# marc345/Dense2Sparse-ViT

Hardware: AMD Instinct MI355X
Metric: training images/s, DeiT-S 224 keep_ratio=0.5 (dense-to-sparse ViT train step, teacher fwd + student fwd/bwd + AdamW) (higher is better)
Workload: dtype f32; 1 GPU; DeiT-Small 224x224 patch16, 1-stage prune keep_ratio=0.5 @ block 3 (196->98 tokens), large LN predictor, kl_div mask loss, per-GPU batch 128; global_batch=128, parallelism=dp1

## Files before the change

dense2sparse-vit_amd/csrc/attention_f32.hip:

```cpp
#include "d2s_common.h"

namespace {

#ifdef D2S_ATTN_STAMPS
__device__ unsigned long long g_attn_stamps[16 * 8192];
#define ASTAMP(i) if (threadIdx.x == 0) { const int L_ = blockIdx.y * gridDim.x + blockIdx.x; if (L_ < 8192) g_attn_stamps[16 * L_ + (i)] = __builtin_amdgcn_s_memtime(); }
#define ASTAMPR(i) if (threadIdx.x == 0) { const int L_ = blockIdx.y * gridDim.x + blockIdx.x; if (L_ < 8192) g_attn_stamps[16 * L_ + (i)] = __builtin_amdgcn_s_memrealtime(); }
#else
#define ASTAMP(i)
#define ASTAMPR(i)
#endif

constexpr int DH = 64;
constexpr int PITCH = 68;

__device__ __forceinline__ void load_rows_regs(const float* __restrict__ base, long ld, int row, int nrows, int half,
                                               float scale, f32x4 (&r)[8]) {
    if (row < nrows) {
        const float* p = base + (long)row * ld + 4 * half;
#pragma unroll
        for (int t = 0; t < 8; ++t) {
            r[t] = *reinterpret_cast<const f32x4*>(p + 8 * t);
#pragma unroll
            for (int j = 0; j < 4; ++j) r[t][j] *= scale;
        }
    } else {
#pragma unroll
        for (int t = 0; t < 8; ++t) r[t] = f32x4{0.f, 0.f, 0.f, 0.f};
    }
}

__device__ __forceinline__ void tile_load(const float* __restrict__ base, long ld, int row0, int nrows, int tid, f32x4 (&r)[2]) {
#pragma unroll
    for (int i = 0; i < 2; ++i) {
        const int f = tid + i * 256, row = row0 + (f >> 4), d4 = (f & 15) * 4;
        r[i] = row < nrows ? *reinterpret_cast<const f32x4*>(base + (long)row * ld + d4) : f32x4{0.f, 0.f, 0.f, 0.f};
    }
}
__device__ __forceinline__ void tile_store(float* __restrict__ S, int tid, const f32x4 (&r)[2]) {
#pragma unroll
    for (int i = 0; i < 2; ++i) {
        const int f = tid + i * 256;
        *reinterpret_cast<f32x4*>(&S[(f >> 4) * PITCH + (f & 15) * 4]) = r[i];
    }
}

__device__ __forceinline__ void mma_lds_reg(const float* __restrict__ S, int l31, int half, const f32x4 (&y)[8], f32x16& acc) {
#pragma unroll
    for (int t = 0; t < 8; ++t) {
        const f32x4 a = *reinterpret_cast<const f32x4*>(&S[l31 * PITCH + 8 * t + 4 * half]);
#pragma unroll
        for (int j = 0; j < 4; ++j) acc = mfma32(a[j], y[t][j], acc);
    }
}
__device__ __forceinline__ void mma_reg_lds(const f32x16& p, const float* __restrict__ S, int l31, int half, f32x16 (&o)[2],
                                            int groups = 4) {
#pragma unroll
    for (int g = 0; g < 4; ++g) {
        if (g < groups) {
#pragma unroll
            for (int r = 4 * g; r < 4 * g + 4; ++r) {
                const float* row = &S[mfma32_row(r, half) * PITCH];
                o[0] = mfma32(p[r], row[l31], o[0]);
                o[1] = mfma32(p[r], row[32 + l31], o[1]);
            }
        }
    }
}

__device__ __forceinline__ void mma_lds_reg_t(const f32x16& p, const float* __restrict__ S, int l31, int half, f32x16 (&o)[2],
                                              int groups = 4) {
#pragma unroll
    for (int g = 0; g < 4; ++g) {
        if (g < groups) {
#pragma unroll
            for (int r = 4 * g; r < 4 * g + 4; ++r) {
                const float* row = &S[mfma32_row(r, half) * PITCH];
                o[0] = mfma32(row[l31], p[r], o[0]);
                o[1] = mfma32(row[32 + l31], p[r], o[1]);
            }
        }
    }
}

struct AttnFwdArgs {
    const float* qkv; float* out; float* lse; float* cls_row;
    const float* policy; float* cinv; const int* cu;
    int n, H; float scale, eps; int total;
};

template <bool POLICY, bool VARLEN>
__global__ __launch_bounds__(256, 3) void attn_fwd_kernel(AttnFwdArgs a) {
    __shared__ __attribute__((aligned(16))) float Ks[32 * PITCH];
    __shared__ __attribute__((aligned(16))) float Vs[32 * PITCH];
    __shared__ float pol_s[32];
    __shared__ __attribute__((aligned(16))) float vred[POLICY ? 16 * 64 : 4];
    __shared__ float vsum_s[64];
    extern __shared__ __attribute__((aligned(16))) float cls_s[];
    const int tid = threadIdx.x, lane = tid & 63, wave = tid >> 6, half = lane >> 5, l31 = lane & 31;
    const int H = a.H;
    ASTAMP(0); ASTAMPR(8);
    int bx, by;
    xcd_remap_2d(bx, by);
    const int b = by / H, h = by % H;
    const long ld = 3L * H * DH;
    const int row_base = VARLEN ? a.cu[b] : 0;
    const int n = VARLEN ? a.cu[b + 1] - row_base : a.n;
    if (VARLEN && bx * 128 >= n) return;
    const long tok0 = VARLEN ? (long)row_base : (long)b * n;
    const float* qb = a.qkv + tok0 * ld + h * DH;
    const float* kb = qb + (long)H * DH;
    const float* vb = kb + (long)H * DH;
    const float* polb = POLICY ? a.policy + (long)b * n : nullptr;
    const float scale = a.scale;
    const int q0 = bx * 128 + wave * 32;
    const bool active = q0 < n;
    const bool want_cls = a.cls_row != nullptr && bx == 0 && wave == 0;
    const int qi = q0 + l31;

    f32x4 qreg[8];
    load_rows_regs(qb, ld, qi, n, half, scale, qreg);

    f32x16 o[2];
#pragma unroll
    for (int r = 0; r < 16; ++r) { o[0][r] = 0.f; o[1][r] = 0.f; }
    float m_run = -INFINITY, l_run = 0.f;
    f32x4 vacc = {0.f, 0.f, 0.f, 0.f};

    const int ntiles = (n + 31) / 32;
    f32x4 kr[2], vr[2];
    float pr = 0.f;
    tile_load(kb, ld, 0, n, tid, kr);
    tile_load(vb, ld, 0, n, tid, vr);
    if (POLICY && tid < 32) pr = tid < n ? polb[tid] : 0.f;
    for (int t = 0; t < ntiles; ++t) {
        __syncthreads();
        tile_store(Ks, tid, kr);
        tile_store(Vs, tid, vr);
        if (POLICY) {
            if (tid < 32) pol_s[tid] = pr;
            vacc += vr[0];
            vacc += vr[1];
        }
        __syncthreads();
        if (t == 0) { ASTAMP(1); }
        if (t == 1) { ASTAMP(2); }
        if (t == 2) { ASTAMP(3); }
        if (t + 1 < ntiles) {
            tile_load(kb, ld, (t + 1) * 32, n, tid, kr);
            tile_load(vb, ld, (t + 1) * 32, n, tid, vr);
            if (POLICY && tid < 32) { const int kj = (t + 1) * 32 + tid; pr = kj < n ? polb[kj] : 0.f; }
        }
        if (!active) continue;
        f32x16 s;
#pragma unroll
        for (int r = 0; r < 16; ++r) s[r] = 0.f;
        mma_lds_reg(Ks, l31, half, qreg, s);
        const int kv0 = t * 32;
        float mt = -INFINITY;
#pragma unroll
        for (int r = 0; r < 16; ++r) {
            if (kv0 + mfma32_row(r, half) >= n) s[r] = -INFINITY;
            mt = fmaxf(mt, s[r]);
        }
        if (want_cls && l31 == 0) {
#pragma unroll
            for (int r = 0; r < 16; ++r) {
                const int key = kv0 + mfma32_row(r, half);
                if (key < n) cls_s[key] = s[r];
            }
        }
        mt = fmaxf(mt, __shfl_xor(mt, 32, 64));
        const float m_new = fmaxf(m_run, mt);
        const float alpha = __expf(m_run - m_new);
        float rs = 0.f;
#pragma unroll
        for (int r = 0; r < 16; ++r) {
            s[r] = __expf(s[r] - m_new);
            if (POLICY) {
                const int kr_ = mfma32_row(r, half);
                s[r] *= (kv0 + kr_ == qi) ? 1.f : pol_s[kr_];
            }
            rs += s[r];
        }
        rs += __shfl_xor(rs, 32, 64);
        l_run = l_run * alpha + rs;
        m_run = m_new;
#pragma unroll
        for (int r = 0; r < 16; ++r) {
            o[0][r] *= alpha;
            o[1][r] *= alpha;
        }
        mma_lds_reg_t(s, Vs, l31, half, o, min(4, (n - kv0 + 7) >> 3));
    }
    ASTAMP(4);
    const float c = POLICY ? a.eps / (float)n : 0.f;
    if (POLICY) {
        *reinterpret_cast<f32x4*>(&vred[(tid >> 4) * 64 + (tid & 15) * 4]) = vacc;
        __syncthreads();
        if (tid < 64) {
            float t = 0.f;
#pragma unroll
            for (int g = 0; g < 16; ++g) t += vred[g * 64 + tid];
            vsum_s[tid] = t * c;
        }
        __syncthreads();
    }
    if (!active) return;
    const float inv_l = 1.0f / (POLICY ? l_run + a.eps : l_run);
    if (qi < n) {
        float* p = a.out + (tok0 + qi) * H * DH + h * DH;
#pragma unroll
        for (int dt = 0; dt < 2; ++dt)
#pragma unroll
            for (int g = 0; g < 4; ++g) {
                f32x4 v;
#pragma unroll
                for (int j = 0; j < 4; ++j) {
                    float num = o[dt][4 * g + j];
                    if (POLICY) num += vsum_s[32 * dt + 8 * g + 4 * half + j];
                    v[j] = num * inv_l;
                }
                *reinterpret_cast<f32x4*>(p + 32 * dt + 8 * g + 4 * half) = v;
            }
    }
    const long stat0 = VARLEN ? (long)h * a.total + row_base : ((long)b * H + h) * n;
    if (half == 0 && qi < n) {
        if (a.lse) a.lse[stat0 + qi] = m_run + logf(POLICY ? l_run + a.eps : l_run);
        if (POLICY && a.cinv) a.cinv[stat0 + qi] = c * inv_l;
    }
    if (want_cls) {
        const float m0 = __shfl(m_run, 0, 64), il0 = __shfl(inv_l, 0, 64);
        float* cr = a.cls_row + stat0;
        for (int j = lane; j < n; j += 64) {
            float e = expf(cls_s[j] - m0);
            if (POLICY) e = e * (j == 0 ? 1.f : polb[j]) + c;
            cr[j] = e * il0;
        }
    }
    ASTAMP(5); ASTAMPR(9);
}

__global__ __launch_bounds__(256) void attn_delta_kernel(const float* __restrict__ out, const float* __restrict__ dout,
                                                         float* __restrict__ delta, long rows, int n, int H) {
    const int lane = threadIdx.x & 63;
    const long row = (long)blockIdx.x * 4 + (threadIdx.x >> 6);
    if (row >= rows) return;
    const long b = row / n, i = row - b * n;
    for (int h = 0; h < H; ++h) {
        const long e = row * H * DH + h * DH + lane;
        const float s = wave_sum(out[e] * dout[e]);
        if (lane == 0) delta[(b * H + h) * n + i] = s;
    }
}

template <bool POLICY>
__global__ __launch_bounds__(256, 3) void attn_bwd_dq_kernel(const float* __restrict__ qkv, const float* __restrict__ dout,
                                                          const float* __restrict__ lse, const float* __restrict__ delta,
                                                          float* __restrict__ dqkv, int n, int H, float scale,
                                                          const float* __restrict__ policy) {
    __shared__ __attribute__((aligned(16))) float Ks[32 * PITCH];
    __shared__ __attribute__((aligned(16))) float Vs[32 * PITCH];
    __shared__ float pol_s[32];
    const int tid = threadIdx.x, lane = tid & 63, wave = tid >> 6, half = lane >> 5, l31 = lane & 31;
    int bx, by;
    xcd_remap_2d(bx, by);
    const int b = by / H, h = by % H;
    const long ld = 3L * H * DH, ldo = (long)H * DH;
    const float* qb = qkv + (long)b * n * ld + h * DH;
    const float* kb = qb + (long)H * DH;
    const float* vb = kb + (long)H * DH;
    const float* dob = dout + (long)b * n * ldo + h * DH;
    const int q0 = bx * 128 + wave * 32;
    const bool active = q0 < n;

    f32x4 qreg[8], doreg[8];
    load_rows_regs(qb, ld, q0 + l31, n, half, scale, qreg);
    load_rows_regs(dob, ldo, q0 + l31, n, half, 1.0f, doreg);
    const bool qok = q0 + l31 < n;
    const float lse_i = qok ? lse[((long)b * H + h) * n + q0 + l31] : INFINITY;
    const float dl_i = qok ? delta[((long)b * H + h) * n + q0 + l31] : 0.f;

    f32x16 dq[2];
#pragma unroll
    for (int r = 0; r < 16; ++r) { dq[0][r] = 0.f; dq[1][r] = 0.f; }

    const int ntiles = (n + 31) / 32;
    f32x4 kr[2], vr[2];
    float pr = 0.f;
    const float* polb = POLICY ? policy + (long)b * n : nullptr;
    tile_load(kb, ld, 0, n, tid, kr);
    tile_load(vb, ld, 0, n, tid, vr);
    if (POLICY && tid < 32) pr = tid < n ? polb[tid] : 0.f;
    for (int t = 0; t < ntiles; ++t) {
        __syncthreads();
        tile_store(Ks, tid, kr);
        tile_store(Vs, tid, vr);
        if (POLICY && tid < 32) pol_s[tid] = pr;
        __syncthreads();
        if (t + 1 < ntiles) {
            tile_load(kb, ld, (t + 1) * 32, n, tid, kr);
            tile_load(vb, ld, (t + 1) * 32, n, tid, vr);
            if (POLICY && tid < 32) { const int kj = (t + 1) * 32 + tid; pr = kj < n ? polb[kj] : 0.f; }
        }
        if (!active) continue;
        f32x16 s, dp;
#pragma unroll
        for (int r = 0; r < 16; ++r) { s[r] = 0.f; dp[r] = 0.f; }
        mma_lds_reg(Ks, l31, half, qreg, s);
        mma_lds_reg(Vs, l31, half, doreg, dp);
        const int kv0 = t * 32;
#pragma unroll
        for (int r = 0; r < 16; ++r) {
            const int kr_ = mfma32_row(r, half);
            float p = (kv0 + kr_ < n) ? __expf(s[r] - lse_i) : 0.f;
            if (POLICY) p *= (kv0 + kr_ == q0 + l31) ? 1.f : pol_s[kr_];
            s[r] = p * (dp[r] - dl_i);
        }
        mma_reg_lds(s, Ks, l31, half, dq, min(4, (n - kv0 + 7) >> 3));
    }
    if (!active) return;
    float* dqb = dqkv + (long)b * n * ld + h * DH;
#pragma unroll
    for (int r = 0; r < 16; ++r) {
        const int qi = q0 + mfma32_row(r, half);
        if (qi < n) {
            float* p = dqb + (long)qi * ld;
            p[l31] = dq[0][r] * scale;
            p[32 + l31] = dq[1][r] * scale;
        }
    }
}

template <bool POLICY>
__global__ __launch_bounds__(256, 2) void attn_bwd_dkv_kernel(const float* __restrict__ qkv, const float* __restrict__ dout,
                                                           const float* __restrict__ lse, const float* __restrict__ delta,
                                                           float* __restrict__ dqkv, int n, int H, float scale,
                                                           const float* __restrict__ policy, const float* __restrict__ cinv) {
    __shared__ __attribute__((aligned(16))) float Qs[32 * PITCH];
    __shared__ __attribute__((aligned(16))) float Ds[32 * PITCH];
    __shared__ float lse_s[32], dl_s[32], ci_s[32];
    const int tid = threadIdx.x, lane = tid & 63, wave = tid >> 6, half = lane >> 5, l31 = lane & 31;
    int bx, by;
    xcd_remap_2d(bx, by);
    const int b = by / H, h = by % H;
    const long ld = 3L * H * DH, ldo = (long)H * DH;
    const float* qb = qkv + (long)b * n * ld + h * DH;
    const float* kb = qb + (long)H * DH;
    const float* vb = kb + (long)H * DH;
    const float* dob = dout + (long)b * n * ldo + h * DH;
    const float* lse_b = lse + ((long)b * H + h) * n;
    const float* dl_b = delta + ((long)b * H + h) * n;
    const int k0 = bx * 128 + wave * 32;
    const bool active = k0 < n;

    f32x4 kreg[8], vreg[8];
    load_rows_regs(kb, ld, k0 + l31, n, half, scale, kreg);
    load_rows_regs(vb, ld, k0 + l31, n, half, 1.0f, vreg);

    f32x16 dk[2], dv[2];
#pragma unroll
    for (int r = 0; r < 16; ++r) { dk[0][r] = 0.f; dk[1][r] = 0.f; dv[0][r] = 0.f; dv[1][r] = 0.f; }

    const int ntiles = (n + 31) / 32;
    f32x4 qr[2], dr[2];
    float lr = 0.f, dlr = 0.f, cir = 0.f;
    const float* ci_b = POLICY ? cinv + ((long)b * H + h) * n : nullptr;
    const float pol_key = (POLICY && k0 + l31 < n) ? policy[(long)b * n + k0 + l31] : 0.f;
    tile_load(qb, ld, 0, n, tid, qr);
    tile_load(dob, ldo, 0, n, tid, dr);
    if (tid < 32) { lr = tid < n ? lse_b[tid] : INFINITY; dlr = tid < n ? dl_b[tid] : 0.f; if (POLICY) cir = tid < n ? ci_b[tid] : 0.f; }
    for (int t = 0; t < ntiles; ++t) {
        __syncthreads();
        tile_store(Qs, tid, qr);
        tile_store(Ds, tid, dr);
        if (tid < 32) { lse_s[tid] = lr; dl_s[tid] = dlr; if (POLICY) ci_s[tid] = cir; }
        __syncthreads();
        if (t + 1 < ntiles) {
            tile_load(qb, ld, (t + 1) * 32, n, tid, qr);
            tile_load(dob, ldo, (t + 1) * 32, n, tid, dr);
            if (tid < 32) {
                const int qi = (t + 1) * 32 + tid;
                lr = qi < n ? lse_b[qi] : INFINITY;
                dlr = qi < n ? dl_b[qi] : 0.f;
                if (POLICY) cir = qi < n ? ci_b[qi] : 0.f;
            }
        }
        if (!active) continue;
        f32x16 s, dp;
#pragma unroll
        for (int r = 0; r < 16; ++r) { s[r] = 0.f; dp[r] = 0.f; }
        mma_lds_reg(Qs, l31, half, kreg, s);
        mma_lds_reg(Ds, l31, half, vreg, dp);
#pragma unroll
        for (int r = 0; r < 16; ++r) {
            const int qi = mfma32_row(r, half);
            float p = __expf(s[r] - lse_s[qi]);
            if (POLICY) p *= (t * 32 + qi == k0 + l31) ? 1.f : pol_key;
            s[r] = POLICY ? p + ci_s[qi] : p;
            dp[r] = p * (dp[r] - dl_s[qi]);
        }
        const int qgroups = min(4, (n - t * 32 + 7) >> 3);
        mma_reg_lds(s, Ds, l31, half, dv, qgroups);
        mma_reg_lds(dp, Qs, l31, half, dk, qgroups);
    }
    if (!active) return;
    float* dkb = dqkv + (long)b * n * ld + (long)H * DH + h * DH;
    float* dvb = dkb + (long)H * DH;
#pragma unroll
    for (int r = 0; r < 16; ++r) {
        const int ki = k0 + mfma32_row(r, half);
        if (ki < n) {
            float* pk = dkb + (long)ki * ld;
            float* pv = dvb + (long)ki * ld;
            pk[l31] = dk[0][r] * scale;
            pk[32 + l31] = dk[1][r] * scale;
            pv[l31] = dv[0][r];
            pv[32 + l31] = dv[1][r];
        }
    }
}

}

#ifdef D2S_ATTN_STAMPS
extern "C" int d2s_debug_read_attn_stamps(unsigned long long* host_out, int n_wg) {
    return hipMemcpyFromSymbol(host_out, HIP_SYMBOL(g_attn_stamps), (size_t)n_wg * 16 * sizeof(unsigned long long)) == hipSuccess ? 0 : -1;
}
#endif

extern "C" {

int d2s_attn_fwd_f32(const float* qkv, float* out, float* lse, float* cls_row, int B, int n, int H, float scale,
                     hipStream_t stream) {
    if (!qkv || !out || !lse || B <= 0 || n <= 0 || H <= 0 || n > 8192) return D2S_ERR_ARG;
    dim3 grid((n + 127) / 128, B * H), block(256);
    AttnFwdArgs a{qkv, out, lse, cls_row, nullptr, nullptr, nullptr, n, H, scale, 0.f, 0};
    hipLaunchKernelGGL((attn_fwd_kernel<false, false>), grid, block, cls_row ? (size_t)n * sizeof(float) : 0, stream, a);
    return d2s_check_launch();
}

int d2s_attn_policy_fwd_f32(const float* qkv, const float* policy, float* out, float* lse, float* cinv, float* cls_row, int B, int n,
                            int H, float scale, float eps, hipStream_t stream) {
    if (!qkv || !policy || !out || !lse || !cinv || B <= 0 || n <= 0 || H <= 0 || n > 8192) return D2S_ERR_ARG;
    dim3 grid((n + 127) / 128, B * H), block(256);
    AttnFwdArgs a{qkv, out, lse, cls_row, policy, cinv, nullptr, n, H, scale, eps, 0};
    hipLaunchKernelGGL((attn_fwd_kernel<true, false>), grid, block, cls_row ? (size_t)n * sizeof(float) : 0, stream, a);
    return d2s_check_launch();
}

int d2s_attn_varlen_fwd_f32(const float* qkv, const int* cu_seqlens, float* out, float* cls_row, int B, int total, int max_n, int H,
                            float scale, hipStream_t stream) {
    if (!qkv || !cu_seqlens || !out || B <= 0 || total <= 0 || max_n <= 0 || max_n > 8192 || H <= 0) return D2S_ERR_ARG;
    dim3 grid((max_n + 127) / 128, B * H), block(256);
    AttnFwdArgs a{qkv, out, nullptr, cls_row, nullptr, nullptr, cu_seqlens, 0, H, scale, 0.f, total};
    hipLaunchKernelGGL((attn_fwd_kernel<false, true>), grid, block, cls_row ? (size_t)max_n * sizeof(float) : 0, stream, a);
    return d2s_check_launch();
}

int d2s_attn_delta(const float* out, const float* dout, float* delta, int B, int n, int H, hipStream_t stream) {
    if (!out || !dout || !delta || B <= 0 || n <= 0 || H <= 0) return D2S_ERR_ARG;
    const long rows = (long)B * n;
    hipLaunchKernelGGL(attn_delta_kernel, dim3((unsigned)((rows + 3) / 4)), dim3(256), 0, stream, out, dout, delta, rows, n, H);
    return d2s_check_launch();
}

int d2s_attn_bwd_f32(const float* qkv, const float* out, const float* dout, const float* lse, float* dqkv, float* delta_ws, int B,
                     int n, int H, float scale, hipStream_t stream) {
    if (!qkv || !out || !dout || !lse || !dqkv || !delta_ws || B <= 0 || n <= 0 || H <= 0) return D2S_ERR_ARG;
    const long rows = (long)B * n;
    hipLaunchKernelGGL(attn_delta_kernel, dim3((unsigned)((rows + 3) / 4)), dim3(256), 0, stream, out, dout, delta_ws, rows, n, H);
    dim3 grid((n + 127) / 128, B * H), block(256);
    hipLaunchKernelGGL(attn_bwd_dq_kernel<false>, grid, block, 0, stream, qkv, dout, lse, delta_ws, dqkv, n, H, scale,
                       static_cast<const float*>(nullptr));
    hipLaunchKernelGGL(attn_bwd_dkv_kernel<false>, grid, block, 0, stream, qkv, dout, lse, delta_ws, dqkv, n, H, scale,
                       static_cast<const float*>(nullptr), static_cast<const float*>(nullptr));
    return d2s_check_launch();
}

int d2s_attn_bwd_dq_f32(const float* qkv, const float* dout, const float* lse, const float* delta_ws, float* dqkv, int B, int n, int H,
                        float scale, hipStream_t stream) {
    if (!qkv || !dout || !lse || !dqkv || !delta_ws || B <= 0 || n <= 0 || H <= 0) return D2S_ERR_ARG;
    dim3 grid((n + 127) / 128, B * H), block(256);
    hipLaunchKernelGGL(attn_bwd_dq_kernel<false>, grid, block, 0, stream, qkv, dout, lse, delta_ws, dqkv, n, H, scale,
                       static_cast<const float*>(nullptr));
    return d2s_check_launch();
}
int d2s_attn_bwd_dkv_f32(const float* qkv, const float* dout, const float* lse, const float* delta_ws, float* dqkv, int B, int n, int H,
                         float scale, hipStream_t stream) {
    if (!qkv || !dout || !lse || !dqkv || !delta_ws || B <= 0 || n <= 0 || H <= 0) return D2S_ERR_ARG;
    dim3 grid((n + 127) / 128, B * H), block(256);
    hipLaunchKernelGGL(attn_bwd_dkv_kernel<false>, grid, block, 0, stream, qkv, dout, lse, delta_ws, dqkv, n, H, scale,
                       static_cast<const float*>(nullptr), static_cast<const float*>(nullptr));
    return d2s_check_launch();
}

int d2s_attn_policy_bwd_f32(const float* qkv, const float* policy, const float* out, const float* dout, const float* lse,
                            const float* cinv, float* dqkv, float* delta_ws, int B, int n, int H, float scale, hipStream_t stream) {
    if (!qkv || !policy || !out || !dout || !lse || !cinv || !dqkv || !delta_ws || B <= 0 || n <= 0 || H <= 0) return D2S_ERR_ARG;
    const long rows = (long)B * n;
    hipLaunchKernelGGL(attn_delta_kernel, dim3((unsigned)((rows + 3) / 4)), dim3(256), 0, stream, out, dout, delta_ws, rows, n, H);
    dim3 grid((n + 127) / 128, B * H), block(256);
    hipLaunchKernelGGL(attn_bwd_dq_kernel<true>, grid, block, 0, stream, qkv, dout, lse, delta_ws, dqkv, n, H, scale, policy);
    hipLaunchKernelGGL(attn_bwd_dkv_kernel<true>, grid, block, 0, stream, qkv, dout, lse, delta_ws, dqkv, n, H, scale, policy, cinv);
    return d2s_check_launch();
}

}
```

Before: 3594 images/s.

## Add single-block short-sequence attention fwd/bwd kernels for n<=256

Adds specialized attention kernels used when sequence length is at most 256 (the ViT case: 197 and 99 tokens). The forward launches one workgroup per (batch, head) with one wave per 32-query tile, sharing K/V tiles through LDS with register prefetch. The backward fuses the delta computation, dK/dV, and dQ into a single kernel that keeps all of K in LDS and assigns dQ chains to idle waves, replacing three launches and redundant K/Q reloads. It is enabled by default via an env toggle; the trade-off is fewer, larger workgroups (less grid parallelism) and high LDS use per block.

```diff
diff --git a/dense2sparse-vit_amd/csrc/attention_f32.hip b/dense2sparse-vit_amd/csrc/attention_f32.hip
--- a/dense2sparse-vit_amd/csrc/attention_f32.hip
+++ b/dense2sparse-vit_amd/csrc/attention_f32.hip
@@ -1,4 +1,6 @@
 #include "d2s_common.h"
+
+#include <type_traits>
 
 namespace {
 
@@ -421,6 +423,297 @@
     }
 }
 
+constexpr int SHORT_MAX_N = 256;
+
+template <int NT>
+__device__ __forceinline__ void tile_load_n(const float* __restrict__ base, long ld, int row0, int nrows, int tid, f32x4 (&r)[512 / NT]) {
+#pragma unroll
+    for (int i = 0; i < 512 / NT; ++i) {
+        const int f = tid + i * NT, row = row0 + (f >> 4), d4 = (f & 15) * 4;
+        r[i] = row < nrows ? *reinterpret_cast<const f32x4*>(base + (long)row * ld + d4) : f32x4{0.f, 0.f, 0.f, 0.f};
+    }
+}
+template <int NT>
+__device__ __forceinline__ void tile_store_n(float* __restrict__ S, int tid, const f32x4 (&r)[512 / NT]) {
+#pragma unroll
+    for (int i = 0; i < 512 / NT; ++i) {
+        const int f = tid + i * NT;
+        *reinterpret_cast<f32x4*>(&S[(f >> 4) * PITCH + (f & 15) * 4]) = r[i];
+    }
+}
+
+template <int NW>
+__global__ __launch_bounds__(NW * 64, NW == 8 ? 4 : 3) void attn_fwd_short_kernel(AttnFwdArgs a) {
+    constexpr int NT = NW * 64, PER = 512 / NT;
+    __shared__ __attribute__((aligned(16))) float Ks[32 * PITCH];
+    __shared__ __attribute__((aligned(16))) float Vs[32 * PITCH];
+    __shared__ float cls_s[SHORT_MAX_N];
+    const int tid = threadIdx.x, lane = tid & 63, wave = tid >> 6, half = lane >> 5, l31 = lane & 31;
+    const int H = a.H, n = a.n;
+    int bx, by;
+    xcd_remap_2d(bx, by);
+    const int b = by / H, h = by % H;
+    const long ld = 3L * H * DH;
+    const long tok0 = (long)b * n;
+    const float* qb = a.qkv + tok0 * ld + h * DH;
+    const float* kb = qb + (long)H * DH;
+    const float* vb = kb + (long)H * DH;
+    const float scale = a.scale;
+    const int q0 = wave * 32;
+    const bool active = q0 < n;
+    const bool want_cls = a.cls_row != nullptr && wave == 0;
+    const int qi = q0 + l31;
+
+    f32x4 qreg[8];
+    load_rows_regs(qb, ld, qi, n, half, scale, qreg);
+
+    f32x16 o[2];
+#pragma unroll
+    for (int r = 0; r < 16; ++r) { o[0][r] = 0.f; o[1][r] = 0.f; }
+    float m_run = -INFINITY, l_run = 0.f;
+
+    const int ntiles = (n + 31) / 32;
+    f32x4 kr[PER], vr[PER];
+    tile_load_n<NT>(kb, ld, 0, n, tid, kr);
+    tile_load_n<NT>(vb, ld, 0, n, tid, vr);
+    for (int t = 0; t < ntiles; ++t) {
+        __syncthreads();
+        tile_store_n<NT>(Ks, tid, kr);
+        tile_store_n<NT>(Vs, tid, vr);
+        __syncthreads();
+        if (t + 1 < ntiles) {
+            tile_load_n<NT>(kb, ld, (t + 1) * 32, n, tid, kr);
+            tile_load_n<NT>(vb, ld, (t + 1) * 32, n, tid, vr);
+        }
+        if (!active) continue;
+        f32x16 s;
+#pragma unroll
+        for (int r = 0; r < 16; ++r) s[r] = 0.f;
+        mma_lds_reg(Ks, l31, half, qreg, s);
+        const int kv0 = t * 32;
+        float mt = -INFINITY;
+#pragma unroll
+        for (int r = 0; r < 16; ++r) {
+            if (kv0 + mfma32_row(r, half) >= n) s[r] = -INFINITY;
+            mt = fmaxf(mt, s[r]);
+        }
+        if (want_cls && l31 == 0) {
+#pragma unroll
+            for (int r = 0; r < 16; ++r) {
+                const int key = kv0 + mfma32_row(r, half);
+                if (key < n) cls_s[key] = s[r];
+            }
+        }
+        mt = fmaxf(mt, __shfl_xor(mt, 32, 64));
+        const float m_new = fmaxf(m_run, mt);
+        const float alpha = __expf(m_run - m_new);
+        float rs = 0.f;
+#pragma unroll
+        for (int r = 0; r < 16; ++r) {
+            s[r] = __expf(s[r] - m_new);
+            rs += s[r];
+        }
+        rs += __shfl_xor(rs, 32, 64);
+        l_run = l_run * alpha + rs;
+        m_run = m_new;
+#pragma unroll
+        for (int r = 0; r < 16; ++r) {
+            o[0][r] *= alpha;
+            o[1][r] *= alpha;
+        }
+        mma_lds_reg_t(s, Vs, l31, half, o, min(4, (n - kv0 + 7) >> 3));
+    }
+    if (!active) return;
+    const float inv_l = 1.0f / l_run;
+    if (qi < n) {
+        float* p = a.out + (tok0 + qi) * H * DH + h * DH;
+#pragma unroll
+        for (int dt = 0; dt < 2; ++dt)
+#pragma unroll
+            for (int g = 0; g < 4; ++g) {
+                f32x4 v;
+#pragma unroll
+                for (int j = 0; j < 4; ++j) v[j] = o[dt][4 * g + j] * inv_l;
+                *reinterpret_cast<f32x4*>(p + 32 * dt + 8 * g + 4 * half) = v;
+            }
+    }
+    const long stat0 = ((long)b * H + h) * n;
+    if (half == 0 && qi < n) a.lse[stat0 + qi] = m_run + logf(l_run);
+    if (want_cls) {
+        const float m0 = __shfl(m_run, 0, 64), il0 = __shfl(inv_l, 0, 64);
+        float* cr = a.cls_row + stat0;
+        for (int j = lane; j < n; j += 64) cr[j] = expf(cls_s[j] - m0) * il0;
+    }
+}
+
+template <int KMAX>
+__global__ __launch_bounds__(512, 2) void attn_bwd_short_kernel(const float* __restrict__ qkv, const float* __restrict__ out,
+                                                                const float* __restrict__ dout, const float* __restrict__ lse,
+                                                                float* __restrict__ dqkv, int n, int H, float scale) {
+    constexpr int NT = 512;
+    constexpr int DSP = KMAX + 8;
+    __shared__ __attribute__((aligned(16))) float Kall[KMAX * PITCH];
+    __shared__ __attribute__((aligned(16))) float dS_s[2][32 * DSP];
+    __shared__ __attribute__((aligned(16))) float Qs[32 * PITCH];
+    __shared__ __attribute__((aligned(16))) float Ds[32 * PITCH];
+    __shared__ float lse_s[32], dl_s[32];
+    const int tid = threadIdx.x, lane = tid & 63, wave = tid >> 6, half = lane >> 5, l31 = lane & 31;
+    int bx, by;
+    xcd_remap_2d(bx, by);
+    const int b = by / H, h = by % H;
+    const long ld = 3L * H * DH, ldo = (long)H * DH;
+    const float* qb = qkv + (long)b * n * ld + h * DH;
+    const float* kb = qb + (long)H * DH;
+    const float* vb = kb + (long)H * DH;
+    const float* dob = dout + (long)b * n * ldo + h * DH;
+    const float* ob = out + (long)b * n * ldo + h * DH;
+    const float* lse_b = lse + ((long)b * H + h) * n;
+    const int ntiles = (n + 31) / 32;
+    const int k0 = wave * 32;
+    const bool active = k0 < n;
+    const bool key_ok = k0 + l31 < n;
+    const int cw0 = ntiles <= 6 ? ntiles : 7, cw1 = ntiles <= 6 ? ntiles + 1 : (ntiles == 7 ? 7 : 6);
+    const bool chain0 = wave == cw0, chain1 = wave == cw1;
+
+#pragma unroll
+    for (int i = 0; i < KMAX / 32; ++i) {
+        const int f = tid + i * NT, row = f >> 4, d4 = (f & 15) * 4;
+        const f32x4 v = row < n ? *reinterpret_cast<const f32x4*>(kb + (long)row * ld + d4) : f32x4{0.f, 0.f, 0.f, 0.f};
+        *reinterpret_cast<f32x4*>(&Kall[row * PITCH + d4]) = v;
+    }
+    f32x4 vreg[8];
+    load_rows_regs(vb, ld, k0 + l31, n, half, 1.0f, vreg);
+
+    f32x16 dk[2], dv[2];
+#pragma unroll
+    for (int r = 0; r < 16; ++r) { dk[0][r] = 0.f; dk[1][r] = 0.f; dv[0][r] = 0.f; dv[1][r] = 0.f; }
+
+    f32x4 qr[1], dr[1];
+    float o_d[4], do_d[4];
+    float lr = 0.f;
+    auto load_tile = [&](int t) {
+        tile_load_n<NT>(qb, ld, t * 32, n, tid, qr);
+        tile_load_n<NT>(dob, ldo, t * 32, n, tid, dr);
+#pragma unroll
+        for (int rr = 0; rr < 4; ++rr) {
+            const int row = t * 32 + 4 * wave + rr;
+            o_d[rr] = row < n ? ob[(long)row * ldo + lane] : 0.f;
+            do_d[rr] = row < n ? dob[(long)row * ldo + lane] : 0.f;
+        }
+        if (tid < 32) { const int qi = t * 32 + tid; lr = qi < n ? lse_b[qi] : INFINITY; }
+    };
+    load_tile(0);
+    __syncthreads();
+    f32x4 kreg[8];
+#pragma unroll
+    for (int t = 0; t < 8; ++t) {
+        kreg[t] = *reinterpret_cast<const f32x4*>(&Kall[min(k0 + l31, KMAX - 1) * PITCH + 8 * t + 4 * half]);
+#pragma unroll
+        for (int j = 0; j < 4; ++j) kreg[t][j] *= scale;
+    }
+
+    float* dqb = dqkv + (long)b * n * ld + h * DH;
+    auto dq_chains = [&](int i, auto d0, auto d1) {
+        constexpr bool D0 = decltype(d0)::value, D1 = decltype(d1)::value;
+        const float* dsb = dS_s[i & 1];
+        f32x16 dq[2];
+#pragma unroll
+        for (int r = 0; r < 16; ++r) { dq[0][r] = 0.f; dq[1][r] = 0.f; }
+        auto group = [&](int kt, int g) {
+            const f32x4 a = *reinterpret_cast<const f32x4*>(&dsb[l31 * DSP + kt * 32 + 8 * g + 4 * half]);
+            float b0[4], b1[4];
+#pragma unroll
+            for (int j = 0; j < 4; ++j) {
+                const float* krow = &Kall[(kt * 32 + 8 * g + 4 * half + j) * PITCH];
+                if (D0) b0[j] = krow[l31];
+                if (D1) b1[j] = krow[32 + l31];
+            }
+#pragma unroll
+            for (int j = 0; j < 4; ++j) {
+                if (D0) dq[0] = mfma32(a[j], b0[j], dq[0]);
+                if (D1) dq[1] = mfma32(a[j], b1[j], dq[1]);
+            }
+        };
+        for (int kt = 0; kt + 1 < ntiles; ++kt) {
+#pragma unroll
+            for (int g = 0; g < 4; ++g) group(kt, g);
+        }
+        const int groups = min(4, (n - (ntiles - 1) * 32 + 7) >> 3);
+        for (int g = 0; g < groups; ++g) group(ntiles - 1, g);
+#pragma unroll
+        for (int r = 0; r < 16; ++r) {
+            const int qi = i * 32 + mfma32_row(r, half);
+            if (qi < n) {
+                float* p = dqb + (long)qi * ld;
+                if (D0) p[l31] = dq[0][r] * scale;
+                if (D1) p[32 + l31] = dq[1][r] * scale;
+            }
+        }
+    };
+    using T_ = std::true_type;
+    using F_ = std::false_type;
+    auto chains = [&](int i) {
+        if (chain0 && chain1) dq_chains(i, T_{}, T_{});
+        else if (chain0) dq_chains(i, T_{}, F_{});
+        else if (chain1) dq_chains(i, F_{}, T_{});
+    };
+
+    for (int t = 0; t < ntiles; ++t) {
+        tile_store_n<NT>(Qs, tid, qr);
+        tile_store_n<NT>(Ds, tid, dr);
+#pragma unroll
+        for (int rr = 0; rr < 4; ++rr) {
+            const float s = wave_sum(o_d[rr] * do_d[rr]);
+            if (lane == 0) dl_s[4 * wave + rr] = s;
+        }
+        if (tid < 32) lse_s[tid] = lr;
+        __syncthreads();
+        if (t + 1 < ntiles) load_tile(t + 1);
+        if (active) {
+            f32x16 s, dp;
+#pragma unroll
+            for (int r = 0; r < 16; ++r) { s[r] = 0.f; dp[r] = 0.f; }
+            mma_lds_reg(Qs, l31, half, kreg, s);
+            mma_lds_reg(Ds, l31, half, vreg, dp);
+            float* dsb = dS_s[t & 1];
+#pragma unroll
+            for (int r = 0; r < 16; ++r) {
+                const int qi = mfma32_row(r, half);
+                const float p = key_ok ? __expf(s[r] - lse_s[qi]) : 0.f;
+                s[r] = p;
+                dp[r] = p * (dp[r] - dl_s[qi]);
+                dsb[qi * DSP + k0 + l31] = dp[r];
+            }
+            const int qgroups = min(4, (n - t * 32 + 7) >> 3);
+            mma_reg_lds(s, Ds, l31, half, dv, qgroups);
+            mma_reg_lds(dp, Qs, l31, half, dk, qgroups);
+        }
+        if (t > 0) chains(t - 1);
+        __syncthreads();
+    }
+    chains(ntiles - 1);
+    if (!active) return;
+    float* dkb = dqkv + (long)b * n * ld + (long)H * DH + h * DH;
+    float* dvb = dkb + (long)H * DH;
+#pragma unroll
+    for (int r = 0; r < 16; ++r) {
+        const int ki = k0 + mfma32_row(r, half);
+        if (ki < n) {
+            float* pk = dkb + (long)ki * ld;
+            float* pv = dvb + (long)ki * ld;
+            pk[l31] = dk[0][r] * scale;
+            pk[32 + l31] = dk[1][r] * scale;
+            pv[l31] = dv[0][r];
+            pv[32 + l31] = dv[1][r];
+        }
+    }
+}
+
+bool attn_short(int n) {
+    static const int on = [] { const char* e = getenv("D2S_ATTN_SHORT"); return e ? atoi(e) : 1; }();
+    return on != 0 && n <= SHORT_MAX_N;
+}
+
 }
 
 #ifdef D2S_ATTN_STAMPS
@@ -434,8 +727,13 @@
 int d2s_attn_fwd_f32(const float* qkv, float* out, float* lse, float* cls_row, int B, int n, int H, float scale,
                      hipStream_t stream) {
     if (!qkv || !out || !lse || B <= 0 || n <= 0 || H <= 0 || n > 8192) return D2S_ERR_ARG;
+    AttnFwdArgs a{qkv, out, lse, cls_row, nullptr, nullptr, nullptr, n, H, scale, 0.f, 0};
+    if (attn_short(n)) {
+        if (n <= 128) hipLaunchKernelGGL(attn_fwd_short_kernel<4>, dim3(1, B * H), dim3(256), 0, stream, a);
+        else hipLaunchKernelGGL(attn_fwd_short_kernel<8>, dim3(1, B * H), dim3(512), 0, stream, a);
+        return d2s_check_launch();
+    }
     dim3 grid((n + 127) / 128, B * H), block(256);
-    AttnFwdArgs a{qkv, out, lse, cls_row, nullptr, nullptr, nullptr, n, H, scale, 0.f, 0};
     hipLaunchKernelGGL((attn_fwd_kernel<false, false>), grid, block, cls_row ? (size_t)n * sizeof(float) : 0, stream, a);
     return d2s_check_launch();
 }
@@ -468,6 +766,11 @@
 int d2s_attn_bwd_f32(const float* qkv, const float* out, const float* dout, const float* lse, float* dqkv, float* delta_ws, int B,
                      int n, int H, float scale, hipStream_t stream) {
     if (!qkv || !out || !dout || !lse || !dqkv || !delta_ws || B <= 0 || n <= 0 || H <= 0) return D2S_ERR_ARG;
+    if (attn_short(n)) {
+        if (n <= 128) hipLaunchKernelGGL(attn_bwd_short_kernel<128>, dim3(1, B * H), dim3(512), 0, stream, qkv, out, dout, lse, dqkv, n, H, scale);
+        else hipLaunchKernelGGL(attn_bwd_short_kernel<256>, dim3(1, B * H), dim3(512), 0, stream, qkv, out, dout, lse, dqkv, n, H, scale);
+        return d2s_check_launch();
+    }
     const long rows = (long)B * n;
     hipLaunchKernelGGL(attn_delta_kernel, dim3((unsigned)((rows + 3) / 4)), dim3(256), 0, stream, out, dout, delta_ws, rows, n, H);
     dim3 grid((n + 127) / 128, B * H), block(256);
```

Result: no change. 3610 images/s, median of 6 (+0.4%).
